# LuoGroup2023/PanTax

Hardware: AMD Instinct MI355X
Metric: PAO wall-time (s) + Mreads/s: packed reads + DB (graphs and their unique-trio index) resident in HBM -> abundance tables; the metric's own GAF -> abundance quantity is value_gaf_to_tables (files -> tables, never `value`) (higher is better)
Workload: dtype int64+f64

## Files before the change

### pantax_amd/csrc/cov_device.hpp

```cpp
#pragma once
#include "common.hpp"
#include "wave.hpp"

namespace ptx {

constexpr int COV_BLOCK = 256;

__device__ __forceinline__ uint32_t bm_peek(const uint32_t *p) {
    return __hip_atomic_load(p, __ATOMIC_RELAXED, __HIP_MEMORY_SCOPE_AGENT);
}
constexpr uint32_t COV_BWIN = 2048;
constexpr int COV_WIN = 2048;
extern __shared__ uint32_t s_cov[];
#define S_WIN(i) s_cov[(i)]
#define S_BM(bmo, i) s_cov[(bmo) + (i)]
#define S_FULL(bmo, i) reinterpret_cast<uint8_t *>(s_cov + (bmo) + COV_BWIN)[(i)]
__host__ __device__ constexpr size_t cov_lds_bytes(int win) { return (size_t)win * 4 + COV_BWIN * 4 + (size_t)win; }
__device__ __forceinline__ void lds_or(uint32_t *__restrict__ bm, uint32_t bmo, uint64_t bw0, uint32_t bwn, uint64_t w, uint32_t m) {
    const uint64_t off = w - bw0;
    if (off < bwn) {
        if ((S_BM(bmo, off) & m) != m) atomicOr(&S_BM(bmo, off), m);
    } else if ((bm_peek(&bm[w]) & m) != m) atomicOr(&bm[w], m);
}
__device__ __forceinline__ void mark_range(uint32_t *__restrict__ bm, uint32_t bmo, uint64_t bw0, uint32_t bwn, uint64_t g0, uint64_t g1) {
    if (g1 <= g0) return;
    uint64_t w0 = g0 >> 5, w1 = (g1 - 1) >> 5;
    uint32_t m0 = 0xFFFFFFFFu << (g0 & 31);
    uint32_t m1 = 0xFFFFFFFFu >> (31 - (uint32_t)((g1 - 1) & 31));
    if (w0 == w1) lds_or(bm, bmo, bw0, bwn, w0, m0 & m1);
    else {
        lds_or(bm, bmo, bw0, bwn, w0, m0);
        for (uint64_t w = w0 + 1; w < w1; ++w) lds_or(bm, bmo, bw0, bwn, w, 0xFFFFFFFFu);
        lds_or(bm, bmo, bw0, bwn, w1, m1);
    }
}
__device__ __forceinline__ void win_or(uint32_t bmo, uint32_t w, uint32_t m) { if ((S_BM(bmo, w) & m) != m) atomicOr(&S_BM(bmo, w), m); }
__device__ __forceinline__ void mark_window(uint32_t bmo, uint32_t r0, uint32_t r1) {
    if (r1 <= r0) return;
    const uint32_t w0 = r0 >> 5, w1 = (r1 - 1) >> 5;
    const uint32_t m0 = 0xFFFFFFFFu << (r0 & 31), m1 = 0xFFFFFFFFu >> (31 - ((r1 - 1) & 31));
    if (w0 == w1) win_or(bmo, w0, m0 & m1);
    else {
        win_or(bmo, w0, m0);
        for (uint32_t w = w0 + 1; w < w1; ++w) win_or(bmo, w, 0xFFFFFFFFu);
        win_or(bmo, w1, m1);
    }
}

constexpr uint32_t STEP_LONG = 0x80u;
constexpr uint32_t STEP_START = 0x40u, STEP_PAD = 0xFFu, STEP_DIST = 0x3Fu;
__device__ __forceinline__ unsigned long long ballot1(bool b) { return __builtin_amdgcn_ballot_w64(b); }
__device__ __forceinline__ bool any1(bool b) { return __builtin_amdgcn_ballot_w64(b) != 0ull; }
__device__ __forceinline__ bool none1(bool b) { return __builtin_amdgcn_ballot_w64(b) == 0ull; }
__device__ __forceinline__ uint32_t slot_in_group(uint32_t group_first_slot, uint32_t code, int lane) {
    const unsigned long long starts = ballot1((code != STEP_PAD) & ((code & STEP_START) != 0u)) & ~1ull;
    const uint32_t below = __builtin_amdgcn_mbcnt_hi((uint32_t)(starts >> 32), __builtin_amdgcn_mbcnt_lo((uint32_t)starts, 0u));
    return group_first_slot + below + (uint32_t)((starts >> lane) & 1ull);
}

__device__ __forceinline__ uint32_t rl_from_memory(uint32_t j, uint32_t b, const uint32_t *__restrict__ node_id, const uint8_t *__restrict__ step_dup,
                                                   uint32_t delta, const uint4 *__restrict__ node_rec, uint32_t len0, uint32_t ps) {
    const uint32_t idj = node_id[b + j];
    if (j == 0 || ((step_dup[b + j] & 1u) && idj == node_id[b])) return len0 - ps;
    return node_rec[idj + delta].z;
}

#ifdef COV_ABLATE
#define ABL(bit) (ablate & (bit))
#else
#define ABL(bit) false
#endif
constexpr int COV_WIN_BACK = 128;
constexpr uint32_t NO_SLOT = 0xFFFFFFFFu;

__device__ __forceinline__ void add_bases(unsigned long long *__restrict__ bases, uint32_t wlo, uint32_t win_n, uint32_t v, uint32_t aln) {
    const uint32_t off = v - wlo;
    if (off < win_n && aln < (1u << 18)) atomicAdd(&S_WIN(off), aln);
    else atomicAdd(&bases[v], (unsigned long long)aln);
}
constexpr uint32_t NO_FULL = 0xFFFFFFFFu;
__device__ __forceinline__ void mark_full_wave(uint32_t *__restrict__ full, uint32_t wlo, uint32_t win_n, uint32_t v) {
    const uint32_t off = v - wlo;
    const bool have = v != NO_FULL;
    if (have && off < win_n) S_FULL(COV_WIN, off) = 1;
    const bool out = have && off >= win_n;
    unsigned long long todo = __ballot(out);
    const uint32_t w = v >> 5, bit = 1u << (v & 31);
    const int lane = threadIdx.x & 63;
    while (todo) {
        const int leader = __builtin_ctzll(todo);
        const uint32_t wl = (uint32_t)__builtin_amdgcn_readlane((int)w, leader);
        const bool mine = out && w == wl;
        const uint32_t orv = wave_reduce(mine ? bit : 0u, [](uint32_t x, uint32_t y) { return x | y; });
        if (lane == leader) atomicOr(&full[wl], orv);
        todo &= ~__ballot(mine);
    }
}

constexpr uint32_t COV_ITEM_GROUPS = 128;
struct __attribute__((packed, aligned(4))) EntPair { uint32_t a, b, c, d; };
constexpr int COV_BLK_SHIFT = 11;

template <int WIN>
__device__ __forceinline__ void mark_full_out_wave(uint32_t *__restrict__ full, bool out, uint32_t v) {
    unsigned long long todo = ballot1(out);
    const uint32_t w = v >> 5, bit = 1u << (v & 31);
    const int lane = threadIdx.x & 63;
    while (todo) {
        const int leader = __builtin_ctzll(todo);
        const uint32_t wl = (uint32_t)__builtin_amdgcn_readlane((int)w, leader);
        const bool mine = out & (w == wl);
        const uint32_t orv = wave_reduce(mine ? bit : 0u, [](uint32_t x, uint32_t y) { return x | y; });
        if (lane == leader) atomicOr(&full[wl], orv);
        todo &= ~ballot1(mine);
    }
}

}
```

### pantax_amd/csrc/stage_cov.hip

```cpp
#include <chrono>
#include <cstdio>
#include <cstdlib>
#include "common.hpp"
#include "primitives.hpp"
#include "wave.hpp"
#include "cov_plan.hpp"
#include "cov_device.hpp"
#pragma clang diagnostic ignored "-Wbitwise-instead-of-logical"

namespace ptx {

template <bool WITH_TRIO, int U, int PASSES, int WIN, bool LONG = false>
__global__ void __launch_bounds__(COV_BLOCK) coverage_fast_kernel(
    const uint2 *__restrict__ items, const uint32_t *__restrict__ group_slot, const uint4 *__restrict__ read_rec, const uint2 *__restrict__ slot_rec,
    const uint32_t *__restrict__ node_id, const uint8_t *__restrict__ step_code, const uint8_t *__restrict__ active,
    const uint4 *__restrict__ node_rec, const uint64_t *__restrict__ bit_off, uint64_t V, unsigned long long *__restrict__ bases,
    uint32_t *__restrict__ bitmap, uint32_t *__restrict__ full, const uint2 *__restrict__ trio_ent, unsigned long long *__restrict__ trio_bases,
    unsigned long long *__restrict__ n_abort, uint32_t ablate, int blk_shift,
    const uint32_t *__restrict__ long_sum = nullptr, const uint32_t *__restrict__ long_len0 = nullptr, uint32_t only_long = 0u,
    uint32_t chunk_groups = 0u, uint32_t total_groups = 0u, uint32_t win_back = 0u, const uint32_t *__restrict__ item_sel = nullptr) {
    constexpr int WAVES = COV_BLOCK / 64;
    const int lane = threadIdx.x & 63, wave = threadIdx.x >> 6;
    uint32_t g0, n_groups;
    if constexpr (LONG) { g0 = blockIdx.x * chunk_groups; n_groups = min(g0 + chunk_groups, total_groups); }
    else { const uint2 item = items[item_sel ? item_sel[blockIdx.x] : blockIdx.x]; g0 = item.x; n_groups = item.y; }
    for (int i = threadIdx.x; i < (int)(cov_lds_bytes(WIN) / 4); i += COV_BLOCK) s_cov[i] = 0;
    uint32_t wlo = 0, win_n = 0, mark_n = 0, bit0_lo = 0, bwn = 0;
    uint64_t bw0 = 0;
#pragma unroll 1
    for (uint32_t g = g0; g < n_groups && win_n == 0; ++g) {
        const uint32_t gs = group_slot[g];
        if (gs == NO_SLOT) continue;
        const uint2 sr0 = slot_rec[gs];
        if ((int)sr0.x < 0 || !active[sr0.x]) continue;
        const uint32_t id0 = node_id[(uint64_t)g * 64], v0 = id0 + sr0.y, in_blk = id0 & ((1u << blk_shift) - 1u);
        const uint32_t back = LONG ? win_back : in_blk + 64u;
        wlo = (v0 > back ? v0 - back : 0u) & ~63u;
        win_n = WIN;
        const uint64_t b_lo = bit_off[wlo], b_hi = bit_off[min((uint64_t)wlo + WIN, V)];
        bw0 = b_lo >> 5;
        bit0_lo = (uint32_t)(bw0 << 5);
        bwn = COV_BWIN;
        mark_n = (b_hi - (bw0 << 5) <= (uint64_t)COV_BWIN * 32) ? (uint32_t)min((uint64_t)WIN, V - wlo) : 0u;
    }
    __builtin_amdgcn_fence(__ATOMIC_RELEASE, "workgroup", "local");
    __builtin_amdgcn_s_barrier();
    __builtin_amdgcn_fence(__ATOMIC_ACQUIRE, "workgroup", "local");
#ifndef COV_NO_PREFETCH
    uint32_t n_code[U], n_id[U], n_gs[U];
    {
        const uint32_t gw0 = g0 + (uint32_t)(wave * U);
#pragma unroll
        for (int u = 0; u < U; ++u) {
            const uint32_t g = gw0 + (uint32_t)u < n_groups ? gw0 + (uint32_t)u : (gw0 < n_groups ? gw0 : g0);
            const uint64_t t = (uint64_t)g * 64 + lane;
            n_code[u] = step_code[t]; n_id[u] = node_id[t]; n_gs[u] = group_slot[g];
        }
    }
#endif
#if !defined(COV_NO_PF2) && !defined(COV_NO_PREFETCH)
    constexpr bool PF2 = !LONG;
#else
    constexpr bool PF2 = false;
#endif
    uint32_t c_code[U], c_id[U], c_gs[U];
    uint4 c_rr[U];
    uint2 c_sr[U];
    bool c_run[U];
#pragma unroll
    for (int u = 0; u < U; ++u) c_run[u] = false;
    if constexpr (PF2) {
        const uint32_t gw0 = g0 + (uint32_t)(wave * U), gw1 = gw0 + (uint32_t)(WAVES * U);
#pragma unroll
        for (int u = 0; u < U; ++u) {
            c_code[u] = n_code[u]; c_id[u] = n_id[u]; c_gs[u] = n_gs[u];
            const uint32_t g = gw1 + (uint32_t)u < n_groups ? gw1 + (uint32_t)u : (gw0 < n_groups ? gw0 : g0);
            const uint64_t t = (uint64_t)g * 64 + lane;
            n_code[u] = step_code[t]; n_id[u] = node_id[t]; n_gs[u] = group_slot[g];
            const bool pad0 = c_code[u] == STEP_PAD;
            const bool run0 = (gw0 + (uint32_t)u < n_groups) & any1(!pad0) & none1(!pad0 & ((c_code[u] & STEP_LONG) != 0u));
            const uint32_t sl = slot_in_group(c_gs[u], c_code[u], lane);
            const uint32_t slot = (pad0 | !run0) ? (c_gs[u] == NO_SLOT ? 0u : c_gs[u]) : sl;
            c_rr[u] = read_rec[slot]; c_sr[u] = slot_rec[slot];
            c_run[u] = run0;
        }
    }
#pragma unroll 1
    for (int pass = 0;; ++pass) {
        const uint32_t gw = g0 + (uint32_t)((pass * WAVES + wave) * U);
        if (gw >= n_groups) break;
        uint32_t code[U], id[U], gs[U];
        bool run[U];
        uint4 rr[U];
        uint2 sr[U];
#ifndef COV_NO_PREFETCH
        if constexpr (PF2) {
            const uint32_t gn = gw + (uint32_t)(WAVES * U), g2 = gn + (uint32_t)(WAVES * U);
            uint32_t m_code[U], m_id[U], m_gs[U];
#pragma unroll
            for (int u = 0; u < U; ++u) {
                run[u] = c_run[u];
                code[u] = c_code[u]; id[u] = c_id[u]; gs[u] = c_gs[u]; rr[u] = c_rr[u]; sr[u] = c_sr[u];
                const uint32_t g = g2 + (uint32_t)u < n_groups ? g2 + (uint32_t)u : gw;
                const uint64_t t = (uint64_t)g * 64 + lane;
                m_code[u] = step_code[t]; m_id[u] = node_id[t]; m_gs[u] = group_slot[g];
                const bool padn = n_code[u] == STEP_PAD;
                const bool runn = (gn + (uint32_t)u < n_groups) & any1(!padn) & none1(!padn & ((n_code[u] & STEP_LONG) != 0u));
                const uint32_t sl = slot_in_group(n_gs[u], n_code[u], lane);
                const uint32_t slot = (padn | !runn) ? (n_gs[u] == NO_SLOT ? 0u : n_gs[u]) : sl;
                c_rr[u] = read_rec[slot]; c_sr[u] = slot_rec[slot];
                c_run[u] = runn;
                c_code[u] = n_code[u]; c_id[u] = n_id[u]; c_gs[u] = n_gs[u];
                n_code[u] = m_code[u]; n_id[u] = m_id[u]; n_gs[u] = m_gs[u];
            }
        } else
        {
            const uint32_t gn = gw + (uint32_t)(WAVES * U);
#pragma unroll
            for (int u = 0; u < U; ++u) {
                run[u] = gw + (uint32_t)u < n_groups;
                code[u] = n_code[u]; id[u] = n_id[u]; gs[u] = n_gs[u];
                const uint32_t g = gn + (uint32_t)u < n_groups ? gn + (uint32_t)u : gw;
                const uint64_t t = (uint64_t)g * 64 + lane;
                n_code[u] = step_code[t]; n_id[u] = node_id[t]; n_gs[u] = group_slot[g];
            }
        }
#else
#pragma unroll
        for (int u = 0; u < U; ++u) {
            const uint32_t g = gw + (uint32_t)u;
            run[u] = g < n_groups;
            const uint64_t t = (uint64_t)(run[u] ? g : gw) * 64 + lane;
            code[u] = step_code[t]; id[u] = node_id[t];
            gs[u] = group_slot[run[u] ? g : gw];
        }
#endif
        bool pad[U];
        uint32_t ll0[U], lsum[U];
#pragma unroll
        for (int u = 0; u < U; ++u) {
            pad[u] = code[u] == STEP_PAD;
            if constexpr (!PF2) {
                const bool has_long = any1(!pad[u] & ((code[u] & STEP_LONG) != 0u));
                run[u] = run[u] & any1(!pad[u]) & (LONG ? (has_long | (only_long == 0u)) : !has_long);
            }
            const uint32_t sl = slot_in_group(gs[u], code[u], lane);
            const uint32_t slot = (pad[u] | !run[u]) ? (gs[u] == NO_SLOT ? 0u : gs[u]) : sl;
            if constexpr (!PF2) { rr[u] = read_rec[slot]; sr[u] = slot_rec[slot]; }
            if constexpr (LONG) { ll0[u] = long_len0[slot]; lsum[u] = long_sum[slot]; }
        }
        uint32_t h_id1[U], h_id2[U], h_codes[U];
        if constexpr (LONG) {
#pragma unroll
            for (int u = 0; u < U; ++u) {
                const uint32_t gu = (uint32_t)__builtin_amdgcn_readfirstlane((int)(gw + (uint32_t)u));
                const uint64_t t0 = (uint64_t)(run[u] && gu != 0u ? gu : 1u) * 64;
                h_id1[u] = node_id[t0 - 1]; h_id2[u] = node_id[t0 - 2];
                h_codes[u] = *reinterpret_cast<const uint32_t *>(step_code + t0 - 4);
            }
        }
        uint4 nr[U];
        uint32_t v[U], act[U];
        bool ok[U];
#pragma unroll
        for (int u = 0; u < U; ++u) {
            ok[u] = run[u] & !pad[u] & ((int)sr[u].x >= 0);
            v[u] = ok[u] ? id[u] + sr[u].y : wlo;
            nr[u] = node_rec[v[u]];
            act[u] = active[ok[u] ? sr[u].x : 0u];
        }
        uint32_t idf[U], i0_[U], hv1[U], hv2[U];
        uint4 nrh1[U], nrh2[U];
        if constexpr (LONG) {
#pragma unroll
            for (int u = 0; u < U; ++u) {
                idf[u] = node_id[rr[u].x];
                const uint32_t gbase = (gw + (uint32_t)u) * 64u;
                const bool ok0 = __builtin_amdgcn_readfirstlane((int)ok[u]) != 0;
                i0_[u] = ok0 ? (uint32_t)__builtin_amdgcn_readfirstlane((int)(gbase - rr[u].x)) : 0u;
                const uint32_t delta0 = (uint32_t)__builtin_amdgcn_readfirstlane((int)sr[u].y);
                hv1[u] = i0_[u] >= 1u ? h_id1[u] + delta0 : wlo;
                hv2[u] = i0_[u] >= 2u ? h_id2[u] + delta0 : wlo;
                nrh1[u] = node_rec[hv1[u]]; nrh2[u] = node_rec[hv2[u]];
            }
        }
        uint32_t i_[U], nl[U], len0[U], nh[U], hx[U], tlo[U], thi[U];
        uint2 e0[U], e1[U];
        bool live[U], single[U], dead_read[U], cross[U];
        int dist[U];
#pragma unroll
        for (int u = 0; u < U; ++u) {
            const uint32_t gbase = (gw + (uint32_t)u) * 64u;
            i_[u] = gbase + (uint32_t)lane - rr[u].x;
            ok[u] = ok[u] & (act[u] != 0u);
            nl[u] = ok[u] ? nr[u].z : 0u;
            if constexpr (LONG) {
                dist[u] = (int)min(ok[u] ? i_[u] : 0u, (uint32_t)lane);
                cross[u] = ok[u] & (i_[u] > (uint32_t)lane);
                const uint32_t in_wave = __shfl(nl[u], lane - dist[u]);
                len0[u] = cross[u] ? ll0[u] : in_wave;
            } else
            len0[u] = __shfl(nl[u], lane - (int)i_[u]);
            uint32_t v2 = wave_shr1(wave_shr1(v[u]));
            uint32_t hw1 = wave_shr1(nr[u].w), hy1 = wave_shr1(nr[u].y);
            if constexpr (LONG) {
                v2 = lane == 0 ? hv2[u] : lane == 1 ? hv1[u] : v2;
                hw1 = lane == 0 ? nrh1[u].w : hw1; hy1 = lane == 0 ? nrh1[u].y : hy1;
            }
            single[u] = rr[u].y == 1u;
            dead_read[u] = !single[u] & (rr[u].z > len0[u]);
            live[u] = ok[u] & !dead_read[u] & !(single[u] & (rr[u].w < rr[u].z));
            nh[u] = 0; hx[u] = 0; tlo[u] = 0; thi[u] = 0;
            e0[u] = make_uint2(0u, 0u); e1[u] = e0[u];
            if (WITH_TRIO && !ABL(4u)) {
                hx[u] = hw1;
                tlo[u] = min(v[u], v2); thi[u] = max(v[u], v2);
                nh[u] = (live[u] & (i_[u] >= 2u) & ((nr_filter(hy1) & nr_pair_bit(tlo[u], thi[u])) != 0u)) ? nr_rows(hy1) : 0u;
                const EntPair ep = *reinterpret_cast<const EntPair *>(trio_ent + (nh[u] ? hx[u] : 0u));
                e0[u] = make_uint2(ep.a, ep.b); e1[u] = make_uint2(ep.c, ep.d);
            }
        }
#pragma unroll
        for (int u = 0; u < U; ++u) {
            const uint32_t k = rr[u].y, ps = rr[u].z, pe = rr[u].w, i = i_[u];
            if (any1(ok[u] & dead_read[u] & (i == 0u))) { if (ok[u] & dead_read[u] & (i == 0u)) atomicAdd(n_abort, 1ull); }
            const uint32_t contrib = (live[u] & !single[u]) ? (i == 0u ? nl[u] - ps : nl[u]) : 0u;
            const uint32_t pexcl = wave_incl_scan_dpp(contrib) - contrib;
            uint32_t seen = pexcl - __shfl(pexcl, lane - (LONG ? dist[u] : (int)i));
            if constexpr (LONG) seen = cross[u] ? lsum[u] - ps : seen;
            const uint32_t tgt = pe - ps;
            uint32_t aln = nl[u];
            if (i + 1u == k) aln = ((pe >= ps) & (tgt > seen)) ? tgt - seen : 0u;
            if (i == 0u) aln = single[u] ? tgt : nl[u] - ps;
            const uint32_t sidx = i == 0u ? ps : 0u;
            uint32_t hi = sidx + aln;
            if (hi > nl[u]) hi = nl[u];
            const bool markable = live[u] & (hi > sidx) & !(single[u] & !((ps < pe) & (pe <= nl[u])));
            const uint32_t dupd = code[u] & STEP_DIST;
            bool earlier = dupd != 0u, at_step0 = dupd == i;
            if constexpr (LONG) {
                const bool lc = (code[u] & STEP_LONG) != 0u;
                const uint32_t id_first = cross[u] ? idf[u] : __shfl(id[u], lane - dist[u]);
                earlier = lc ? (code[u] & 1u) != 0u : earlier;
                at_step0 = lc ? id[u] == id_first : at_step0;
            }
            const uint32_t rl = !live[u] ? 0u : !earlier ? aln : (at_step0 ? len0[u] - ps : nl[u]);
            const uint32_t off = v[u] - wlo;
            const bool inw = off < win_n;
            if (live[u] & !earlier & (aln != 0u) && !ABL(2u)) {
                if (inw & (aln < (1u << 18))) atomicAdd(&S_WIN(off), aln);
                else atomicAdd(&bases[v[u]], (unsigned long long)aln);
            }
            const bool whole = markable & (sidx == 0u) & (hi == nl[u]);
            if constexpr (LONG) { if (!ABL(1u) && !ABL(8u)) mark_full_out_wave<WIN>(full, whole & !inw, v[u]); }
            if (markable && !ABL(1u)) {
                if (whole) {
                    if (inw) S_FULL(WIN, off) = 1; else if (!LONG && !ABL(8u)) atomicOr(&full[v[u] >> 5], 1u << (v[u] & 31));
                } else if (off < mark_n) {
                    const uint32_t rel = nr[u].x - bit0_lo;
                    mark_window(WIN, rel + sidx, rel + hi);
                } else if (!ABL(8u)) {
                    const uint64_t bo = nr_bit_off(nr[u]);
                    mark_range(bitmap, WIN, bw0, bwn, bo + sidx, bo + hi);
                }
            }
            if (WITH_TRIO && !ABL(4u)) {
                uint32_t rl1 = wave_shr1(rl), rl2 = wave_shr1(rl1);
                if constexpr (LONG) {
                    const uint32_t idf0 = (uint32_t)__builtin_amdgcn_readfirstlane((int)idf[u]), l0 = (uint32_t)__builtin_amdgcn_readfirstlane((int)len0[u]),
                                   ps0 = (uint32_t)__builtin_amdgcn_readfirstlane((int)ps);
                    const uint32_t c1 = h_codes[u] >> 24, c2 = (h_codes[u] >> 16) & 0xFFu;
                    const uint32_t rlh1 = ((i0_[u] == 1u) | (((c1 & 1u) != 0u) & (h_id1[u] == idf0))) ? l0 - ps0 : nrh1[u].z;
                    const uint32_t rlh2 = ((i0_[u] == 2u) | (((c2 & 1u) != 0u) & (h_id2[u] == idf0))) ? l0 - ps0 : nrh2[u].z;
                    rl2 = lane == 0 ? rlh2 : lane == 1 ? rlh1 : rl2;
                    rl1 = lane == 0 ? rlh1 : rl1;
                }
                constexpr uint32_t NO_ROW = 0xFFFFFFFFu;
                const bool m0 = (nh[u] != 0u) & (e0[u].x == tlo[u]) & (e0[u].y == thi[u]);
                const bool m1 = (nh[u] > 1u) & (e1[u].x == tlo[u]) & (e1[u].y == thi[u]);
                uint32_t row = m0 ? hx[u] : m1 ? hx[u] + 1u : NO_ROW;
                if (any1(!(m0 | m1) & (nh[u] > 2u))) {
                    if (!(m0 | m1) & (nh[u] > 2u))
                        for (uint32_t j = 2; j < nh[u]; ++j) {
                            const uint2 e = trio_ent[hx[u] + j];
                            if (e.x == tlo[u] && e.y == thi[u]) { row = hx[u] + j; break; }
                        }
                }
                const uint32_t sum = rl2 + rl1 + rl;
                if ((row != NO_ROW) & (sum != 0u)) atomicAdd(&trio_bases[row], (unsigned long long)sum);
            }
        }
    }
    __syncthreads();
    if (win_n) {
        for (int i = threadIdx.x; i < WIN; i += COV_BLOCK) {
            const uint32_t c = S_WIN(i);
            if (c) atomicAdd(&bases[wlo + i], (unsigned long long)c);
            const unsigned long long fb = __ballot(S_FULL(WIN, i) != 0);
            if (fb && (lane & 31) == 0 && !ABL(32u)) {
                const uint32_t m = (uint32_t)(fb >> (lane & 32));
                if (m) atomicOr(&full[(wlo + i) >> 5], m);
            }
        }
        if (!ABL(16u))
        for (uint32_t i = threadIdx.x; i < bwn; i += COV_BLOCK) {
            const uint32_t m = S_BM(WIN, i);
            if (m) atomicOr(&bitmap[bw0 + i], m);
        }
    }
}

template <int WS_U, bool EAGER = false>
__global__ void __launch_bounds__(256) walk_sum_kernel(uint64_t T, const uint32_t *__restrict__ group_slot, const uint8_t *__restrict__ step_dup,
                                                       const uint4 *__restrict__ read_rec, const uint2 *__restrict__ slot_rec,
                                                       const uint32_t *__restrict__ node_id, const uint32_t *__restrict__ node_len,
                                                       uint32_t *__restrict__ long_sum, uint32_t *__restrict__ long_len0) {
    const int lane = threadIdx.x & 63;
    const uint64_t stride = (uint64_t)gridDim.x * 256 * WS_U;
    for (uint64_t base = ((uint64_t)blockIdx.x * 256 + (threadIdx.x - lane)) * WS_U; base < T; base += stride) {
        uint32_t code[WS_U], slot[WS_U], id[WS_U], nl[WS_U], gs_e[WS_U], id_e[WS_U];
        uint64_t t[WS_U];
        bool any = false;
#pragma unroll
        for (int u = 0; u < WS_U; ++u) {
            t[u] = base + (uint64_t)u * 64 + lane;
            code[u] = t[u] < T ? step_dup[t[u]] : STEP_PAD;
            if constexpr (EAGER) { gs_e[u] = t[u] < T ? group_slot[t[u] >> 6] : NO_SLOT; id_e[u] = t[u] < T ? node_id[t[u]] : 0u; }
        }
#pragma unroll
        for (int u = 0; u < WS_U; ++u) any = any || (code[u] != STEP_PAD && (code[u] & STEP_LONG));
        if (!__any(any)) continue;
#pragma unroll
        for (int u = 0; u < WS_U; ++u) {
            slot[u] = NO_SLOT; id[u] = 0;
            uint32_t gs;
            if constexpr (EAGER) gs = gs_e[u]; else gs = t[u] < T ? group_slot[t[u] >> 6] : NO_SLOT;
            const uint32_t sl = slot_in_group(gs, code[u], lane);
            if (code[u] != STEP_PAD && (code[u] & STEP_LONG)) { slot[u] = sl; if constexpr (EAGER) id[u] = id_e[u]; else id[u] = node_id[t[u]]; }
        }
        uint2 sr[WS_U];
        uint4 rr[WS_U];
#pragma unroll
        for (int u = 0; u < WS_U; ++u) {
            sr[u] = make_uint2(0xFFFFFFFFu, 0u); rr[u] = make_uint4(0u, 0u, 0u, 0u);
            if (slot[u] != NO_SLOT) { sr[u] = slot_rec[slot[u]]; rr[u] = read_rec[slot[u]]; }
        }
#pragma unroll
        for (int u = 0; u < WS_U; ++u) {
            nl[u] = 0;
            const bool counted = slot[u] != NO_SLOT && (int)sr[u].x >= 0 && (uint32_t)(t[u] - rr[u].x) + 1 < rr[u].y;
            if (counted) nl[u] = node_len[id[u] + sr[u].y];
        }
#pragma unroll
        for (int u = 0; u < WS_U; ++u) {
            if (!__any(slot[u] != NO_SLOT)) continue;
            if (slot[u] != NO_SLOT && (int)sr[u].x >= 0 && (uint32_t)(t[u] - rr[u].x) + 1 < rr[u].y && t[u] == rr[u].x)
                long_len0[slot[u]] = nl[u];
            const uint32_t prev = __shfl_up(slot[u], 1);
            const bool head = lane == 0 || prev != slot[u];
            const unsigned long long heads = __ballot(head);
            const int start = 63 - __builtin_clzll(heads & ((2ull << lane) - 1ull));
            const uint32_t sc = wave_incl_scan_dpp(nl[u]);
            const uint32_t front = __shfl(sc, start > 0 ? start - 1 : 0);
            const uint32_t incl = sc - (start > 0 ? front : 0u);
            const unsigned long long after = heads & ~((2ull << lane) - 1ull);
            const bool tail = after ? (lane + 1 == __builtin_ctzll(after)) : lane == 63;
            if (tail && slot[u] != NO_SLOT && incl) atomicAdd(&long_sum[slot[u]], incl);
        }
    }
}

__global__ void __launch_bounds__(256) popcount_kernel(uint64_t V, const uint64_t *__restrict__ bit_off, const uint32_t *__restrict__ full,
                                                       const uint32_t *__restrict__ bitmap, uint32_t *__restrict__ cov) {
    for (uint64_t v = (uint64_t)blockIdx.x * 256 + threadIdx.x; v < V; v += (uint64_t)gridDim.x * 256) {
        uint64_t g0 = bit_off[v], g1 = bit_off[v + 1];
        uint32_t c = 0;
        if ((full[v >> 5] >> (uint32_t)(v & 31)) & 1u) c = (uint32_t)(g1 - g0);
        else if (g1 > g0) {
            uint64_t w0 = g0 >> 5, w1 = (g1 - 1) >> 5;
            uint32_t m0 = 0xFFFFFFFFu << (g0 & 31);
            uint32_t m1 = 0xFFFFFFFFu >> (31 - (uint32_t)((g1 - 1) & 31));
            if (w0 == w1) c = __popc(bitmap[w0] & m0 & m1);
            else {
                c = __popc(bitmap[w0] & m0);
                for (uint64_t w = w0 + 1; w < w1; ++w) c += __popc(bitmap[w]);
                c += __popc(bitmap[w1] & m1);
            }
        }
        cov[v] = c;
    }
}

constexpr uint32_t PCL_WORDS = 2304;
__global__ void __launch_bounds__(256) popcount_long_kernel(uint64_t V, const uint64_t *__restrict__ bit_off, const uint32_t *__restrict__ full,
                                                            const uint32_t *__restrict__ bitmap, uint32_t *__restrict__ cov) {
    __shared__ __attribute__((aligned(16))) uint32_t s_prefix[4 * PCL_WORDS];
    const uint32_t lane = threadIdx.x & 63, wave = threadIdx.x >> 6;
    uint32_t *pw = s_prefix + wave * PCL_WORDS;
    const uint64_t n_str = (V + 63) / 64;
    for (uint64_t st = (uint64_t)blockIdx.x * 4 + wave; st < n_str; st += (uint64_t)gridDim.x * 4) {
        const uint64_t v = st * 64 + lane;
        const bool in = v < V;
        const uint64_t g0 = in ? bit_off[v] : 0ull, g1 = in ? bit_off[v + 1] : 0ull;
        const uint64_t b0 = __shfl(g0, 0);
        const uint32_t last = (uint32_t)min((uint64_t)63, V - 1 - st * 64);
        const uint64_t b1 = __shfl(g1, (int)last);
        const uint64_t wa = (b0 >> 5) & ~3ull, nw = b1 > b0 ? ((b1 - 1) >> 5) - wa + 1 : 0;
        const bool coop = nw <= (uint64_t)PCL_WORDS && __builtin_amdgcn_ballot_w64(in && g1 - g0 > 64ull) != 0ull;
        if (coop) {
            uint32_t carry = 0;
            for (uint32_t k = 0; k < (uint32_t)nw; k += 256) {
                const uint32_t i = k + 4u * lane;
                const uint4 x = i < (uint32_t)nw ? *reinterpret_cast<const uint4 *>(bitmap + wa + i) : make_uint4(0u, 0u, 0u, 0u);
                const uint32_t p0 = (uint32_t)__popc(x.x), p1 = p0 + (uint32_t)__popc(x.y), p2 = p1 + (uint32_t)__popc(x.z), p3 = p2 + (uint32_t)__popc(x.w);
                const uint32_t incl = wave_incl_scan_dpp(p3);
                const uint32_t base = carry + incl - p3;
                if (i < (uint32_t)nw) *reinterpret_cast<uint4 *>(pw + i) = make_uint4(base, base + p0, base + p1, base + p2);
                carry += (uint32_t)__builtin_amdgcn_readlane((int)incl, 63);
            }
            __builtin_amdgcn_fence(__ATOMIC_RELEASE, "workgroup", "local");
            __builtin_amdgcn_wave_barrier();
            __builtin_amdgcn_fence(__ATOMIC_ACQUIRE, "workgroup", "local");
        }
        uint32_t c = 0;
        if (in && g1 > g0) {
            const uint64_t w0 = g0 >> 5, w1 = (g1 - 1) >> 5;
            const uint32_t m0 = 0xFFFFFFFFu << (g0 & 31), m1 = 0xFFFFFFFFu >> (31 - (uint32_t)((g1 - 1) & 31));
            if ((full[v >> 5] >> (uint32_t)(v & 31)) & 1u) c = (uint32_t)(g1 - g0);
            else if (coop) c = (pw[w1 - wa] + (uint32_t)__popc(bitmap[w1] & m1)) - (pw[w0 - wa] + (uint32_t)__popc(bitmap[w0] & ~m0));
            else if (w0 == w1) c = __popc(bitmap[w0] & m0 & m1);
            else {
                c = __popc(bitmap[w0] & m0);
                for (uint64_t w = w0 + 1; w < w1; ++w) c += __popc(bitmap[w]);
                c += __popc(bitmap[w1] & m1);
            }
        }
        if (coop) __builtin_amdgcn_wave_barrier();
        if (in) cov[v] = c;
    }
}

__global__ void __launch_bounds__(256) count_nonzero_words_kernel(const uint32_t *__restrict__ p, uint64_t n, unsigned long long *__restrict__ out) {
    unsigned long long c = 0;
    for (uint64_t i = (uint64_t)blockIdx.x * 256 + threadIdx.x; i < n; i += (uint64_t)gridDim.x * 256) c += p[i] != 0u;
    if (c) atomicAdd(out, c);
}

int coverage_prepare(Ctx *ctx, Db *db, Reads *rd, bool with_trio) {
    const CovArenaLayout a = cov_arena_layout(db->V, with_trio ? db->U : 0, db->L);
    const size_t off_trio = a.off_trio, off_bm = a.off_bm, off_full = a.off_full, total = a.total;
    PTX_HIP(ctx, db->d_cov_arena.alloc(total));
    uint8_t *base = db->d_cov_arena.p;
    db->d_bases.view(base, db->V);
    db->d_trio_bases.view(base + off_trio, a.n_trio);
    db->d_abort = reinterpret_cast<unsigned long long *>(base + a.off_abort);
    db->d_bitmap.view(base + off_bm, a.words);
    db->d_full.view(base + off_full, a.fwords);
    const uint64_t sig = (uint64_t)(uintptr_t)base ^ ((uint64_t)total * 0x9E3779B97F4A7C15ull) ^ ((uint64_t)off_bm << 1) ^ ((uint64_t)off_full << 2) ^ (uint64_t)off_trio;
    db->cov_arena_total = total;
    if (db->cov_clean_pending) {
        PTX_HIP(ctx, hipStreamWaitEvent(ctx->stream, db->ev_cov_clean, 0));
        db->cov_clean_pending = false;
    }
    if (db->cov_arena_clean && db->cov_arena_sig == sig) {
        if (ctx->cfg.cov_arena_verify) {
            DevBuf<unsigned long long> d_nz;
            PTX_HIP(ctx, d_nz.alloc(1));
            PTX_HIP(ctx, hipMemsetAsync(d_nz.p, 0, 8, ctx->stream));
            PTX_HIP(ctx, hipMemsetAsync(db->d_abort, 0, 8, ctx->stream));
            hipLaunchKernelGGL(count_nonzero_words_kernel, dim3(grid_for(total / 4, 256, ctx->n_cu * 8)), dim3(256), 0, ctx->stream, reinterpret_cast<const uint32_t *>(base), (uint64_t)(total / 4), d_nz.p);
            unsigned long long nz = 0;
            PTX_TRY(download(ctx, &nz, d_nz.p, 1));
            PTX_HIP(ctx, hipStreamSynchronize(ctx->stream));
            if (nz) return fail(ctx, PANTAX_HIP_E_STATE, "coverage_prepare: %llu non-zero words in an arena its last readers should have left clean", nz);
        }
        PTX_HIP(ctx, hipMemsetAsync(db->d_abort, 0, 8, ctx->stream));
    } else {
        KTimer t(ctx, "zero_fill_kernel");
        PTX_TRY(zero_fill(ctx, base, total));
    }
    db->cov_arena_clean = false;
    db->cov_arena_sig = sig;
    if (rd->R && rd->T_pad && rd->n_long && rd->long_sums_db != 0 && rd->long_sums_db == db->uid) {
    } else if (rd->R && rd->T_pad && rd->n_long) {
        PTX_HIP(ctx, hipMemsetAsync(rd->d_long_sum.p, 0, rd->R * sizeof(uint32_t), ctx->stream));
        KTimer t(ctx, "walk_sum_kernel");
        const bool eager = (uint64_t)rd->n_long * 2 > rd->n_slots;
        hipLaunchKernelGGL((eager ? walk_sum_kernel<4, true> : walk_sum_kernel<4, false>), dim3(grid_for(rd->T_pad / 4 + 1, 256, ctx->n_cu * 16)), dim3(256), 0, ctx->stream, rd->T_pad, rd->d_g_group_slot.p,
                           rd->d_g_step_dup.p, rd->d_g_read_rec.p, rd->d_g_slot_rec.p, rd->d_g_node_id.p, db->d_node_len.p, rd->d_long_sum.p,
                           rd->d_long_len0.p);
    }
    PTX_HIP(ctx, hipGetLastError());
    db->cov_prepared = true;
    return 0;
}

int coverage_arena_clean_async(Ctx *ctx, Db *db) {
    if (!db->d_cov_arena.p || !db->cov_arena_total || !ctx->stream2) return 0;
    uint8_t *f_ptr = db->d_cov_arena.p;
    const size_t f_n = db->cov_arena_total;
    if (!db->ev_cov_read) PTX_HIP(ctx, hipEventCreateWithFlags(&db->ev_cov_read, hipEventDisableTiming));
    if (!db->ev_cov_clean) PTX_HIP(ctx, hipEventCreateWithFlags(&db->ev_cov_clean, hipEventDisableTiming));
    PTX_HIP(ctx, hipEventRecord(db->ev_cov_read, ctx->stream));
    PTX_HIP(ctx, hipStreamWaitEvent(ctx->stream2, db->ev_cov_read, 0));
    hipStream_t main_stream = ctx->stream;
    ctx->stream_main = main_stream; ctx->stream = ctx->stream2;
    int rc;
    rc = zero_fill(ctx, f_ptr, f_n);
    const hipError_t e = hipEventRecord(db->ev_cov_clean, ctx->stream2);
    ctx->stream = main_stream; ctx->stream_main = nullptr;
    if (rc != 0) return rc;
    PTX_HIP(ctx, e);
    db->cov_done = false;
    db->cov_arena_clean = true; db->cov_clean_pending = true;
    return 0;
}

struct CovLap {
    Ctx *ctx;
    bool on;
    std::chrono::steady_clock::time_point prev = std::chrono::steady_clock::now();
    void operator()(const char *what) {
        if (!on) return;
        (void)hipStreamSynchronize(ctx->stream);
        const auto now = std::chrono::steady_clock::now();
        std::fprintf(stderr, "[node_coverage]        %-28s %9.3f ms\n", what, std::chrono::duration<double, std::milli>(now - prev).count());
        prev = now;
    }
};

static int active_flags(Ctx *ctx, Db *db, const uint8_t *d_active, const uint8_t **out) {
    if (!d_active) {
        if (db->d_ones.n < db->S) { PTX_HIP(ctx, db->d_ones.alloc(db->S)); PTX_HIP(ctx, hipMemsetAsync(db->d_ones.p, 1, db->S, ctx->stream)); }
        d_active = db->d_ones.p;
    }
    *out = d_active;
    return 0;
}

struct ItemList { uint32_t n; const uint32_t *d; };
static int item_selection(Ctx *ctx, Db *db, const Reads *rd, ItemList *out) {
    *out = {rd->n_items, nullptr};
    if (db->item_sel_layout == rd->layout_id && rd->layout_id != 0) {
        *out = {db->item_sel_n, db->item_sel_on ? db->d_item_sel.p : nullptr};
    } else if (rd->h_item_block.size() == rd->n_items && rd->item_blk_shift > 0 && db->S && !db->h_range_start.empty()) {
        const CovItemSel s = cov_item_select(rd->h_item_block, rd->item_blk_shift, db->h_range_start, db->h_range_end);
        if (s.on && s.n_sel) PTX_TRY(upload(ctx, db->d_item_sel, s.sel.data(), s.sel.size()));
        *out = {s.n_sel, s.on && s.n_sel ? db->d_item_sel.p : nullptr};
        db->item_sel_layout = rd->layout_id; db->item_sel_n = s.n_sel; db->item_sel_on = s.on;
    }
    return 0;
}

struct CovFastTail {
    const uint2 *items; int blk_shift; const uint32_t *long_sum, *long_len0; uint32_t only_long, chunk_groups, total_groups, win_back; const uint32_t *item_sel;
};
template <int U, int PASSES, int WIN, bool LONG>
static void fast_launch_as(Ctx *ctx, Db *db, Reads *rd, const uint8_t *d_act, bool trio, int grid, const CovFastTail &t) {
    if (grid <= 0) return;
    const auto kernel = trio ? coverage_fast_kernel<true, U, PASSES, WIN, LONG> : coverage_fast_kernel<false, U, PASSES, WIN, LONG>;
    hipLaunchKernelGGL(kernel, dim3(grid), dim3(COV_BLOCK), cov_lds_bytes(WIN), ctx->stream, t.items, rd->d_g_group_slot.p, rd->d_g_read_rec.p,
                       rd->d_g_slot_rec.p, rd->d_g_node_id.p, rd->d_g_step_dup.p, d_act, db->d_node_rec.p, db->d_bit_off.p, db->V, db->d_bases.p,
                       db->d_bitmap.p, db->d_full.p, db->d_trio_ent.p, db->d_trio_bases.p, db->d_abort, ctx->cfg.cov_ablate ,
                       t.blk_shift, t.long_sum, t.long_len0, t.only_long, t.chunk_groups, t.total_groups, t.win_back, t.item_sel);
}

static int fast_launch(Ctx *ctx, Db *db, Reads *rd, const uint8_t *d_act, bool trio, const CovFastShape &f, const ItemList &list) {
    const CovFastTail t{rd->d_g_items.p, rd->item_blk_shift, nullptr, nullptr, 0u, 0u, 0u, 0u, list.d};
    const int grid = (int)list.n;
    const auto is = [&](int u, int passes, int win) { return f.u == u && f.passes == passes && f.win == win; };
    if (is(1, 8, 2048)) fast_launch_as<1, 8, 2048, false>(ctx, db, rd, d_act, trio, grid, t);
    else if (is(2, 4, 2048)) fast_launch_as<2, 4, 2048, false>(ctx, db, rd, d_act, trio, grid, t);
    else if (is(2, 8, 2048)) fast_launch_as<2, 8, 2048, false>(ctx, db, rd, d_act, trio, grid, t);
    else if (is(2, 8, 3072)) fast_launch_as<2, 8, 3072, false>(ctx, db, rd, d_act, trio, grid, t);
    else if (is(2, 8, 4096)) fast_launch_as<2, 8, 4096, false>(ctx, db, rd, d_act, trio, grid, t);
    else if (is(2, 4, 3072)) fast_launch_as<2, 4, 3072, false>(ctx, db, rd, d_act, trio, grid, t);
    else if (is(2, 8, 2304)) fast_launch_as<2, 8, 2304, false>(ctx, db, rd, d_act, trio, grid, t);
    else if (is(2, 8, 2560)) fast_launch_as<2, 8, 2560, false>(ctx, db, rd, d_act, trio, grid, t);
    else if (is(2, 4, 2304)) fast_launch_as<2, 4, 2304, false>(ctx, db, rd, d_act, trio, grid, t);
    else if (is(2, 4, 2560)) fast_launch_as<2, 4, 2560, false>(ctx, db, rd, d_act, trio, grid, t);
    else if (is(1, 8, 2304)) fast_launch_as<1, 8, 2304, false>(ctx, db, rd, d_act, trio, grid, t);
    else if (is(4, 4, 2304)) fast_launch_as<4, 4, 2304, false>(ctx, db, rd, d_act, trio, grid, t);
    else if (is(4, 4, 2048)) fast_launch_as<4, 4, 2048, false>(ctx, db, rd, d_act, trio, grid, t);
    else if (is(4, 4, 3072)) fast_launch_as<4, 4, 3072, false>(ctx, db, rd, d_act, trio, grid, t);
    else return fail(ctx, PANTAX_HIP_E_STATE, "coverage_launch: no short-read kernel of shape U = %d, PASSES = %d, WIN = %d", f.u, f.passes, f.win);
    return 0;
}

static int long_launch(Ctx *ctx, Db *db, Reads *rd, const uint8_t *d_act, bool trio, const CovPlan &plan) {
    if (!rd->d_long_sum.p) { PTX_HIP(ctx, rd->d_long_sum.alloc(rd->R)); PTX_HIP(ctx, rd->d_long_len0.alloc(rd->R)); }
    const CovLongShape &l = plan.lng;
    const uint32_t total_groups = (uint32_t)(rd->T_pad / 64);
    const int grid = (int)((total_groups + l.chunk_groups - 1) / l.chunk_groups);
    const CovFastTail t{nullptr, 0, rd->d_long_sum.p, rd->d_long_len0.p, plan.only_long ? 1u : 0u, l.chunk_groups, total_groups, l.win_back, nullptr};
    if (l.u == 1 && l.win == 2048) fast_launch_as<1, 1, 2048, true>(ctx, db, rd, d_act, trio, grid, t);
    else if (l.u == 1 && l.win == 3072) fast_launch_as<1, 1, 3072, true>(ctx, db, rd, d_act, trio, grid, t);
    else if (l.u == 1 && l.win == 4096) fast_launch_as<1, 1, 4096, true>(ctx, db, rd, d_act, trio, grid, t);
    else if (l.u == 2 && l.win == 2048) fast_launch_as<2, 1, 2048, true>(ctx, db, rd, d_act, trio, grid, t);
    else if (l.u == 2 && l.win == 4096) fast_launch_as<2, 1, 4096, true>(ctx, db, rd, d_act, trio, grid, t);
    else if (l.u == 2 && l.win == 3072) fast_launch_as<2, 1, 3072, true>(ctx, db, rd, d_act, trio, grid, t);
    else return fail(ctx, PANTAX_HIP_E_STATE, "coverage_launch: no long-walk kernel of shape U = %d, WIN = %d", l.u, l.win);
    return 0;
}

static int count_launch(Ctx *ctx, Db *db) {
    PTX_HIP(ctx, db->d_cov.alloc(db->V));
    KTimer t(ctx, "popcount_kernel");
    if (long_node_shape(db->L, db->V, ctx->cfg.ncs_prefix_min, ctx->cfg.ncs_no_prefix))
        hipLaunchKernelGGL(popcount_long_kernel, dim3(grid_for((db->V + 63) / 64, 4, ctx->n_cu * 8)), dim3(256), 0, ctx->stream, db->V,
                           db->d_bit_off.p, db->d_full.p, db->d_bitmap.p, db->d_cov.p);
    else
        hipLaunchKernelGGL(popcount_kernel, dim3(grid_for(db->V, 256, ctx->n_cu * 8)), dim3(256), 0, ctx->stream, db->V,
                           db->d_bit_off.p, db->d_full.p, db->d_bitmap.p, db->d_cov.p);
    return 0;
}

int coverage_launch(Ctx *ctx, Db *db, Reads *rd, const uint8_t *d_active, bool with_trio, bool defer_count) {
    if (!rd->grouped) return fail(ctx, PANTAX_HIP_E_STATE, "node_coverage: these reads are a slice kept as plain columns (to be routed to their owner), not resident reads");
    const bool trace = ctx->cfg.trace && !defer_count;
    CovLap lap{ctx, trace};
    if (!db->cov_prepared) PTX_TRY(coverage_prepare(ctx, db, rd, with_trio));
    lap("arena + zero fill");
    db->cov_prepared = false;
    db->cov_stage = false;
    db->trio_free_valid = false;
    const bool trio = with_trio && db->U;
    const uint8_t *d_act_fast = d_active;
    if (rd->R && rd->T_pad) PTX_TRY(active_flags(ctx, db, d_active, &d_act_fast));
    const CtxConfig &cfg = ctx->cfg;
    const CovPlan plan = cov_plan(rd->T_pad, rd->n_long, rd->n_slots, rd->n_items, rd->R, cfg.cov_general, cfg.cov_long, cfg.covf_shape, cfg.covl_shape,
                                  cfg.cov_shape, cfg.cov_xcd);
    if (plan.run_fast) {
        KTimer t(ctx, "coverage_fast_kernel");
        ItemList list;
        PTX_TRY(item_selection(ctx, db, rd, &list));
        if (trace) std::fprintf(stderr, "[node_coverage]        %u of %u items launched\n", list.n, rd->n_items);
        PTX_TRY(fast_launch(ctx, db, rd, d_act_fast, trio, plan.fast, list));
    }
    if (plan.run_long) {
        KTimer t(ctx, "coverage_long_kernel");
        PTX_TRY(long_launch(ctx, db, rd, d_act_fast, trio, plan));
    }
    if (plan.run_step) {
        KTimer t(ctx, "coverage_step_kernel");
        PTX_TRY(coverage_step_launch(ctx, db, rd, d_active, trio, plan));
    }
    PTX_HIP(ctx, hipGetLastError());
    lap("coverage kernels");
    db->cov_count_pending = defer_count && db->V != 0;
    if (db->V && !defer_count) PTX_TRY(count_launch(ctx, db));
    PTX_HIP(ctx, hipGetLastError());
    lap("popcount");
    db->cov_done = true;
    return 0;
}

}
```

Baseline: 6413.

## Cut register pressure in coverage kernel by rematerialising and packing per-step state

Reduces live VGPRs in the coverage fast kernel. It packs per-lane run flags into a bitmask, packs step index, read count and dup distance into one meta word, and recomputes v2 and len0 via lane permutes instead of keeping them across the loop. It also defers far bitmap marking until after the trio lookup, swaps __shfl for direct ds_bpermute, computes lane and wave with wave-uniform intrinsics, and caps SGPRs. Recomputation adds extra cross-lane ops in exchange for the chance of higher occupancy, and a trace-only print reports register and occupancy figures.

```diff
diff --git a/pantax_amd/csrc/cov_device.hpp b/pantax_amd/csrc/cov_device.hpp
--- a/pantax_amd/csrc/cov_device.hpp
+++ b/pantax_amd/csrc/cov_device.hpp
@@ -52,6 +52,7 @@
 __device__ __forceinline__ unsigned long long ballot1(bool b) { return __builtin_amdgcn_ballot_w64(b); }
 __device__ __forceinline__ bool any1(bool b) { return __builtin_amdgcn_ballot_w64(b) != 0ull; }
 __device__ __forceinline__ bool none1(bool b) { return __builtin_amdgcn_ballot_w64(b) == 0ull; }
+__device__ __forceinline__ uint32_t lane_get(uint32_t x, int src) { return (uint32_t)__builtin_amdgcn_ds_bpermute(src << 2, (int)x); }
 __device__ __forceinline__ uint32_t slot_in_group(uint32_t group_first_slot, uint32_t code, int lane) {
     const unsigned long long starts = ballot1((code != STEP_PAD) & ((code & STEP_START) != 0u)) & ~1ull;
     const uint32_t below = __builtin_amdgcn_mbcnt_hi((uint32_t)(starts >> 32), __builtin_amdgcn_mbcnt_lo((uint32_t)starts, 0u));
diff --git a/pantax_amd/csrc/stage_cov.hip b/pantax_amd/csrc/stage_cov.hip
--- a/pantax_amd/csrc/stage_cov.hip
+++ b/pantax_amd/csrc/stage_cov.hip
@@ -1,3 +1,4 @@
+#include <atomic>
 #include <chrono>
 #include <cstdio>
 #include <cstdlib>
@@ -11,7 +12,7 @@
 namespace ptx {
 
 template <bool WITH_TRIO, int U, int PASSES, int WIN, bool LONG = false>
-__global__ void __launch_bounds__(COV_BLOCK) coverage_fast_kernel(
+__global__ void __launch_bounds__(COV_BLOCK) __attribute__((amdgpu_num_sgpr(80))) coverage_fast_kernel(
     const uint2 *__restrict__ items, const uint32_t *__restrict__ group_slot, const uint4 *__restrict__ read_rec, const uint2 *__restrict__ slot_rec,
     const uint32_t *__restrict__ node_id, const uint8_t *__restrict__ step_code, const uint8_t *__restrict__ active,
     const uint4 *__restrict__ node_rec, const uint64_t *__restrict__ bit_off, uint64_t V, unsigned long long *__restrict__ bases,
@@ -20,7 +21,9 @@
     const uint32_t *__restrict__ long_sum = nullptr, const uint32_t *__restrict__ long_len0 = nullptr, uint32_t only_long = 0u,
     uint32_t chunk_groups = 0u, uint32_t total_groups = 0u, uint32_t win_back = 0u, const uint32_t *__restrict__ item_sel = nullptr) {
     constexpr int WAVES = COV_BLOCK / 64;
-    const int lane = threadIdx.x & 63, wave = threadIdx.x >> 6;
+    constexpr bool META = !LONG, V2R = !LONG, L0R = !LONG;
+    const int wave = __builtin_amdgcn_readfirstlane((int)(threadIdx.x >> 6));
+    const int lane = (int)__builtin_amdgcn_mbcnt_hi(~0u, __builtin_amdgcn_mbcnt_lo(~0u, 0u));
     uint32_t g0, n_groups;
     if constexpr (LONG) { g0 = blockIdx.x * chunk_groups; n_groups = min(g0 + chunk_groups, total_groups); }
     else { const uint2 item = items[item_sel ? item_sel[blockIdx.x] : blockIdx.x]; g0 = item.x; n_groups = item.y; }
@@ -66,9 +69,7 @@
     uint32_t c_code[U], c_id[U], c_gs[U];
     uint4 c_rr[U];
     uint2 c_sr[U];
-    bool c_run[U];
-#pragma unroll
-    for (int u = 0; u < U; ++u) c_run[u] = false;
+    uint32_t c_run = 0u;
     if constexpr (PF2) {
         const uint32_t gw0 = g0 + (uint32_t)(wave * U), gw1 = gw0 + (uint32_t)(WAVES * U);
 #pragma unroll
@@ -82,7 +83,7 @@
             const uint32_t sl = slot_in_group(c_gs[u], c_code[u], lane);
             const uint32_t slot = (pad0 | !run0) ? (c_gs[u] == NO_SLOT ? 0u : c_gs[u]) : sl;
             c_rr[u] = read_rec[slot]; c_sr[u] = slot_rec[slot];
-            c_run[u] = run0;
+            c_run |= run0 ? 1u << u : 0u;
         }
     }
 #pragma unroll 1
@@ -97,9 +98,11 @@
         if constexpr (PF2) {
             const uint32_t gn = gw + (uint32_t)(WAVES * U), g2 = gn + (uint32_t)(WAVES * U);
             uint32_t m_code[U], m_id[U], m_gs[U];
+            const uint32_t runs = c_run;
+            c_run = 0u;
 #pragma unroll
             for (int u = 0; u < U; ++u) {
-                run[u] = c_run[u];
+                run[u] = ((runs >> u) & 1u) != 0u;
                 code[u] = c_code[u]; id[u] = c_id[u]; gs[u] = c_gs[u]; rr[u] = c_rr[u]; sr[u] = c_sr[u];
                 const uint32_t g = g2 + (uint32_t)u < n_groups ? g2 + (uint32_t)u : gw;
                 const uint64_t t = (uint64_t)g * 64 + lane;
@@ -109,7 +112,7 @@
                 const uint32_t sl = slot_in_group(n_gs[u], n_code[u], lane);
                 const uint32_t slot = (padn | !runn) ? (n_gs[u] == NO_SLOT ? 0u : n_gs[u]) : sl;
                 c_rr[u] = read_rec[slot]; c_sr[u] = slot_rec[slot];
-                c_run[u] = runn;
+                c_run |= runn ? 1u << u : 0u;
                 c_code[u] = n_code[u]; c_id[u] = n_id[u]; c_gs[u] = n_gs[u];
                 n_code[u] = m_code[u]; n_id[u] = m_id[u]; n_gs[u] = m_gs[u];
             }
@@ -184,7 +187,7 @@
                 nrh1[u] = node_rec[hv1[u]]; nrh2[u] = node_rec[hv2[u]];
             }
         }
-        uint32_t i_[U], nl[U], len0[U], nh[U], hx[U], tlo[U], thi[U];
+        uint32_t i_[U], nl[U], len0[U], nh[U], hx[U], v2_[U], meta[U];
         uint2 e0[U], e1[U];
         bool live[U], single[U], dead_read[U], cross[U];
         int dist[U];
@@ -197,12 +200,12 @@
             if constexpr (LONG) {
                 dist[u] = (int)min(ok[u] ? i_[u] : 0u, (uint32_t)lane);
                 cross[u] = ok[u] & (i_[u] > (uint32_t)lane);
-                const uint32_t in_wave = __shfl(nl[u], lane - dist[u]);
+                const uint32_t in_wave = lane_get(nl[u], lane - dist[u]);
                 len0[u] = cross[u] ? ll0[u] : in_wave;
             } else
-            len0[u] = __shfl(nl[u], lane - (int)i_[u]);
-            uint32_t v2 = wave_shr1(wave_shr1(v[u]));
-            uint32_t hw1 = wave_shr1(nr[u].w), hy1 = wave_shr1(nr[u].y);
+            len0[u] = lane_get(nl[u], lane - (int)i_[u]);
+            uint32_t v2 = wave_shr1z(wave_shr1z(v[u]));
+            uint32_t hw1 = wave_shr1z(nr[u].w), hy1 = wave_shr1z(nr[u].y);
             if constexpr (LONG) {
                 v2 = lane == 0 ? hv2[u] : lane == 1 ? hv1[u] : v2;
                 hw1 = lane == 0 ? nrh1[u].w : hw1; hy1 = lane == 0 ? nrh1[u].y : hy1;
@@ -210,23 +213,34 @@
             single[u] = rr[u].y == 1u;
             dead_read[u] = !single[u] & (rr[u].z > len0[u]);
             live[u] = ok[u] & !dead_read[u] & !(single[u] & (rr[u].w < rr[u].z));
-            nh[u] = 0; hx[u] = 0; tlo[u] = 0; thi[u] = 0;
+            nh[u] = 0; hx[u] = 0; v2_[u] = 0; meta[u] = 0;
+            if constexpr (META) {
+                meta[u] = (i_[u] & 0xFFu) | ((rr[u].y & 0xFFu) << 8) | ((code[u] & STEP_DIST) << 16);
+                asm("" : "+v"(meta[u]));
+            }
             e0[u] = make_uint2(0u, 0u); e1[u] = e0[u];
             if (WITH_TRIO && !ABL(4u)) {
                 hx[u] = hw1;
-                tlo[u] = min(v[u], v2); thi[u] = max(v[u], v2);
-                nh[u] = (live[u] & (i_[u] >= 2u) & ((nr_filter(hy1) & nr_pair_bit(tlo[u], thi[u])) != 0u)) ? nr_rows(hy1) : 0u;
+                if constexpr (!V2R) v2_[u] = v2;
+                else asm("" : "+v"(v[u]));
+                const uint32_t tlo = min(v[u], v2), thi = max(v[u], v2);
+                nh[u] = (live[u] & (i_[u] >= 2u) & ((nr_filter(hy1) & nr_pair_bit(tlo, thi)) != 0u)) ? nr_rows(hy1) : 0u;
                 const EntPair ep = *reinterpret_cast<const EntPair *>(trio_ent + (nh[u] ? hx[u] : 0u));
                 e0[u] = make_uint2(ep.a, ep.b); e1[u] = make_uint2(ep.c, ep.d);
             }
         }
 #pragma unroll
         for (int u = 0; u < U; ++u) {
-            const uint32_t k = rr[u].y, ps = rr[u].z, pe = rr[u].w, i = i_[u];
-            if (any1(ok[u] & dead_read[u] & (i == 0u))) { if (ok[u] & dead_read[u] & (i == 0u)) atomicAdd(n_abort, 1ull); }
+            const bool ab = ok[u] & dead_read[u] & (i_[u] == 0u);
+            if (any1(ab)) { if (ab) atomicAdd(n_abort, 1ull); }
+        }
+#pragma unroll
+        for (int u = 0; u < U; ++u) {
+            const uint32_t ps = rr[u].z, pe = rr[u].w;
+            const uint32_t i = !META ? i_[u] : meta[u] & 0xFFu, k = !META ? rr[u].y : (meta[u] >> 8) & 0xFFu;
             const uint32_t contrib = (live[u] & !single[u]) ? (i == 0u ? nl[u] - ps : nl[u]) : 0u;
             const uint32_t pexcl = wave_incl_scan_dpp(contrib) - contrib;
-            uint32_t seen = pexcl - __shfl(pexcl, lane - (LONG ? dist[u] : (int)i));
+            uint32_t seen = pexcl - lane_get(pexcl, lane - (LONG ? dist[u] : (int)i));
             if constexpr (LONG) seen = cross[u] ? lsum[u] - ps : seen;
             const uint32_t tgt = pe - ps;
             uint32_t aln = nl[u];
@@ -236,15 +250,18 @@
             uint32_t hi = sidx + aln;
             if (hi > nl[u]) hi = nl[u];
             const bool markable = live[u] & (hi > sidx) & !(single[u] & !((ps < pe) & (pe <= nl[u])));
-            const uint32_t dupd = code[u] & STEP_DIST;
+            const uint32_t dupd = !META ? code[u] & STEP_DIST : meta[u] >> 16;
             bool earlier = dupd != 0u, at_step0 = dupd == i;
             if constexpr (LONG) {
                 const bool lc = (code[u] & STEP_LONG) != 0u;
-                const uint32_t id_first = cross[u] ? idf[u] : __shfl(id[u], lane - dist[u]);
+                const uint32_t id_first = cross[u] ? idf[u] : lane_get(id[u], lane - dist[u]);
                 earlier = lc ? (code[u] & 1u) != 0u : earlier;
                 at_step0 = lc ? id[u] == id_first : at_step0;
             }
-            const uint32_t rl = !live[u] ? 0u : !earlier ? aln : (at_step0 ? len0[u] - ps : nl[u]);
+            uint32_t l0 = 0;
+            if constexpr (!L0R) l0 = len0[u];
+            else if (any1(live[u] & earlier & at_step0)) l0 = lane_get(nl[u], lane - (int)i);
+            const uint32_t rl = !live[u] ? 0u : !earlier ? aln : (at_step0 ? l0 - ps : nl[u]);
             const uint32_t off = v[u] - wlo;
             const bool inw = off < win_n;
             if (live[u] & !earlier & (aln != 0u) && !ABL(2u)) {
@@ -253,19 +270,17 @@
             }
             const bool whole = markable & (sidx == 0u) & (hi == nl[u]);
             if constexpr (LONG) { if (!ABL(1u) && !ABL(8u)) mark_full_out_wave<WIN>(full, whole & !inw, v[u]); }
+            bool far_mark = false;
             if (markable && !ABL(1u)) {
                 if (whole) {
                     if (inw) S_FULL(WIN, off) = 1; else if (!LONG && !ABL(8u)) atomicOr(&full[v[u] >> 5], 1u << (v[u] & 31));
                 } else if (off < mark_n) {
                     const uint32_t rel = nr[u].x - bit0_lo;
                     mark_window(WIN, rel + sidx, rel + hi);
-                } else if (!ABL(8u)) {
-                    const uint64_t bo = nr_bit_off(nr[u]);
-                    mark_range(bitmap, WIN, bw0, bwn, bo + sidx, bo + hi);
-                }
+                } else far_mark = !ABL(8u);
             }
             if (WITH_TRIO && !ABL(4u)) {
-                uint32_t rl1 = wave_shr1(rl), rl2 = wave_shr1(rl1);
+                uint32_t rl1 = wave_shr1z(rl), rl2 = wave_shr1z(rl1);
                 if constexpr (LONG) {
                     const uint32_t idf0 = (uint32_t)__builtin_amdgcn_readfirstlane((int)idf[u]), l0 = (uint32_t)__builtin_amdgcn_readfirstlane((int)len0[u]),
                                    ps0 = (uint32_t)__builtin_amdgcn_readfirstlane((int)ps);
@@ -276,24 +291,31 @@
                     rl1 = lane == 0 ? rlh1 : rl1;
                 }
                 constexpr uint32_t NO_ROW = 0xFFFFFFFFu;
-                const bool m0 = (nh[u] != 0u) & (e0[u].x == tlo[u]) & (e0[u].y == thi[u]);
-                const bool m1 = (nh[u] > 1u) & (e1[u].x == tlo[u]) & (e1[u].y == thi[u]);
+                const uint32_t v2 = !V2R ? v2_[u] : wave_shr1z(wave_shr1z(v[u]));
+                const uint32_t tlo = min(v[u], v2), thi = max(v[u], v2);
+                const bool m0 = (nh[u] != 0u) & (e0[u].x == tlo) & (e0[u].y == thi);
+                const bool m1 = (nh[u] > 1u) & (e1[u].x == tlo) & (e1[u].y == thi);
                 uint32_t row = m0 ? hx[u] : m1 ? hx[u] + 1u : NO_ROW;
                 if (any1(!(m0 | m1) & (nh[u] > 2u))) {
                     if (!(m0 | m1) & (nh[u] > 2u))
                         for (uint32_t j = 2; j < nh[u]; ++j) {
                             const uint2 e = trio_ent[hx[u] + j];
-                            if (e.x == tlo[u] && e.y == thi[u]) { row = hx[u] + j; break; }
+                            if (e.x == tlo && e.y == thi) { row = hx[u] + j; break; }
                         }
                 }
                 const uint32_t sum = rl2 + rl1 + rl;
                 if ((row != NO_ROW) & (sum != 0u)) atomicAdd(&trio_bases[row], (unsigned long long)sum);
             }
+            if (far_mark) {
+                const uint64_t bo = nr_bit_off(nr[u]);
+                mark_range(bitmap, WIN, bw0, bwn, bo + sidx, bo + hi);
+            }
         }
     }
     __syncthreads();
     if (win_n) {
-        for (int i = threadIdx.x; i < WIN; i += COV_BLOCK) {
+        const int tid = wave * 64 + lane;
+        for (int i = tid; i < WIN; i += COV_BLOCK) {
             const uint32_t c = S_WIN(i);
             if (c) atomicAdd(&bases[wlo + i], (unsigned long long)c);
             const unsigned long long fb = __ballot(S_FULL(WIN, i) != 0);
@@ -303,7 +325,7 @@
             }
         }
         if (!ABL(16u))
-        for (uint32_t i = threadIdx.x; i < bwn; i += COV_BLOCK) {
+        for (uint32_t i = (uint32_t)tid; i < bwn; i += COV_BLOCK) {
             const uint32_t m = S_BM(WIN, i);
             if (m) atomicOr(&bitmap[bw0 + i], m);
         }
@@ -559,6 +581,19 @@
 static void fast_launch_as(Ctx *ctx, Db *db, Reads *rd, const uint8_t *d_act, bool trio, int grid, const CovFastTail &t) {
     if (grid <= 0) return;
     const auto kernel = trio ? coverage_fast_kernel<true, U, PASSES, WIN, LONG> : coverage_fast_kernel<false, U, PASSES, WIN, LONG>;
+    if (ctx->cfg.trace) {
+        static std::atomic<bool> said[2];
+        if (!said[trio].exchange(true)) {
+            hipFuncAttributes attr{};
+            int per_cu = 0;
+            if (hipFuncGetAttributes(&attr, reinterpret_cast<const void *>(kernel)) == hipSuccess &&
+                hipOccupancyMaxActiveBlocksPerMultiprocessor(&per_cu, kernel, COV_BLOCK, cov_lds_bytes(WIN)) == hipSuccess)
+                std::fprintf(stderr, "[coverage] coverage_fast_kernel<%d,%d,%d,%d,%d>: %d VGPRs, %zu B scratch, %zu B LDS, %d workgroups a CU\n", (int)trio, U, PASSES,
+                             WIN, (int)LONG, attr.numRegs, (size_t)attr.localSizeBytes, (size_t)attr.sharedSizeBytes + cov_lds_bytes(WIN), per_cu);
+            else
+                (void)hipGetLastError();
+        }
+    }
     hipLaunchKernelGGL(kernel, dim3(grid), dim3(COV_BLOCK), cov_lds_bytes(WIN), ctx->stream, t.items, rd->d_g_group_slot.p, rd->d_g_read_rec.p,
                        rd->d_g_slot_rec.p, rd->d_g_node_id.p, rd->d_g_step_dup.p, d_act, db->d_node_rec.p, db->d_bit_off.p, db->V, db->d_bases.p,
                        db->d_bitmap.p, db->d_full.p, db->d_trio_ent.p, db->d_trio_bases.p, db->d_abort, ctx->cfg.cov_ablate ,
```

New measurement: 6498 (median of 6 runs). No clear change (+1.3%).
